# martenlienen/generative-turbulence

Measured on AMD Instinct MI355X. Metric: U-Net fwd+bwd voxels/sec (DDPM training step, 192x64x48x4), higher is better.
Workload: dtype bf16

## Files before the change

generative-turbulence_amd/csrc/tdx_resize.hip:

```cpp
#include "tdx_common.h"
#include <stdlib.h>

struct AxisMap {
    int in, out;
    float scale;
};
__host__ __device__ inline AxisMap make_axis(int in, int out) {
    AxisMap a;
    a.in = in; a.out = out;
    a.scale = out > 1 ? (float)(in - 1) / (float)(out - 1) : 0.0f;
    return a;
}
__host__ __device__ __forceinline__ void axis_taps(const AxisMap& a, int o, int& i0, int& i1, float& w1) {
    const float src = a.scale * (float)o;
    i0 = min((int)src, a.in - 1);
    w1 = fminf(fmaxf(src - (float)i0, 0.0f), 1.0f);
    i1 = i0 + ((i0 + 1 < a.in) ? 1 : 0);
}

struct TileGrid {
    int nx, ny, nz;
    int sy, sz;
    int tx, ty, tz;
};
// ... 184 lines not shown
__host__ __device__ __forceinline__ float axis_weight(const AxisMap& a, int o, int i) {
    int i0, i1;
    float w1;
    axis_taps(a, o, i0, i1, w1);
    float w = 0.f;
    if (i0 == i) w += 1.0f - w1;
    if (i1 == i) w += w1;
    return w;
}
__host__ __device__ __forceinline__ void axis_span(const AxisMap& a, int i, int& first, int& cnt) {
    int lo, hi;
    axis_range(a, i, lo, hi);
    first = hi + 1;
    int last = lo - 1;
    for (int o = lo; o <= hi; ++o)
        if (axis_weight(a, o, i) != 0.f) {
            first = min(first, o);
            last = o;
        }
    cnt = last - first + 1;
    if (cnt < 0) cnt = 0;
}

template <typename T, int K>
__global__ void __launch_bounds__(256)
resize_bwd_kernel(const T* __restrict__ dy, const T* __restrict__ add, T* __restrict__ dx, AxisMap ax, AxisMap ay, AxisMap az,
                  int C, TileGrid tg) {
    __shared__ int s_first[3][RS_MAXT], s_cnt[3][RS_MAXT];
    __shared__ float s_w[3][RS_MAXT][RS_KMAX];
    int b, ix0, iy0, iz0;
    tile_origin(tg, b, ix0, iy0, iz0);
    if (threadIdx.x < 3 * RS_MAXT) {
        const int a = threadIdx.x / RS_MAXT, k = threadIdx.x % RS_MAXT;
        const AxisMap& m = a == 0 ? ax : (a == 1 ? ay : az);
        const int i = min((a == 0 ? ix0 : (a == 1 ? iy0 : iz0)) + k, m.in - 1);
        int f, c;
        axis_span(m, i, f, c);
        s_first[a][k] = f; s_cnt[a][k] = c;
        for (int j = 0; j < RS_KMAX; ++j) s_w[a][k][j] = j < c ? axis_weight(m, f + j, i) : 0.f;
    }
    __syncthreads();
    const int L = C >> 3;
    const int per_pass = 256 / L;
    const int lc = (int)threadIdx.x % L;
    const int nvox = tg.tx * tg.ty * tg.tz;
    if ((int)threadIdx.x >= per_pass * L) return;
    for (int slot = (int)threadIdx.x / L; slot < nvox; slot += per_pass) {
        const int kz = slot & (tg.tz - 1), ky = (slot >> tg.sz) & (tg.ty - 1), kx = slot >> (tg.sz + tg.sy);
        const int ix = ix0 + kx, iy = iy0 + ky, iz = iz0 + kz;
        if (ix >= ax.in || iy >= ay.in || iz >= az.in) continue;
        const int fx = s_first[0][kx], cx = s_cnt[0][kx], fy = s_first[1][ky], cy = s_cnt[1][ky], fz = s_first[2][kz];
        float wz[K];
        int oz[K];
#pragma unroll
        for (int k = 0; k < K; ++k) {
            oz[k] = min(fz + k, az.out - 1);
            wz[k] = s_w[2][kz][k];
        }
        const T* gb = dy + ((int64_t)b * ax.out * ay.out * az.out) * C + lc * 8;
        float acc[8];
#pragma unroll
        for (int j = 0; j < 8; ++j) acc[j] = 0.f;
        for (int a = 0; a < cx; ++a) {
            const float wx = s_w[0][kx][a];
            for (int bb = 0; bb < cy; ++bb) {
                const float wxy = wx * s_w[1][ky][bb];
                const T* row = gb + (((int64_t)(fx + a) * ay.out + (fy + bb)) * az.out) * C;
                Raw8<T> t[K];
#pragma unroll
                for (int k = 0; k < K; ++k) t[k].load(row + (int64_t)oz[k] * C);
                __builtin_amdgcn_sched_barrier(0);
#pragma unroll
                for (int k = 0; k < K; ++k) {
                    const float w = wxy * wz[k];
                    const Vec8<T> v = t[k].get();
#pragma unroll
                    for (int j = 0; j < 8; ++j) acc[j] += w * v.v[j];
                }
            }
        }
        const int64_t di = ((((int64_t)b * ax.in + ix) * ay.in + iy) * az.in + iz) * C + lc * 8;
        if (add != nullptr) {
            Vec8<T> a;
            a.load(add + di);
#pragma unroll
            for (int j = 0; j < 8; ++j) acc[j] += a.v[j];
        }
        Vec8<T> o;
#pragma unroll
        for (int j = 0; j < 8; ++j) o.v[j] = acc[j];
        o.store(dx + di);
    }
}

template <typename T>
__global__ void __launch_bounds__(256)
resize_bwd_generic_kernel(const T* __restrict__ dy, const T* __restrict__ add, T* __restrict__ dx, AxisMap ax, AxisMap ay,
                          AxisMap az, int C, int64_t total) {
    const int L = C >> 3;
    int64_t i = (int64_t)blockIdx.x * blockDim.x + threadIdx.x;
    if (i >= total) return;
    const int lc = (int)(i % L);
    int64_t v = i / L;
    const int iz = (int)(v % az.in); v /= az.in;
    const int iy = (int)(v % ay.in); v /= ay.in;
// ... 65 lines not shown
    const AxisMap mx = make_axis(Xi, Xo), my = make_axis(Yi, Yo), mz = make_axis(Zi, Zo);
    if (C <= 64 && !((tg.tx | tg.ty | tg.tz) & 1) && Xo > Xi && Yo > Yi && Zo > Zi && pair_window_ok(mx) &&
        pair_window_ok(my) && pair_window_ok(mz)) {
        TDX_DISPATCH_DTYPE(dtype, hipLaunchKernelGGL((resize_up_pairs_kernel<T>), dim3((unsigned)blocks), dim3(256), 0,
                                                      as_stream(stream), (const T*)x, (T*)y, mx, my, mz, C, tg));
        return tdx_launch_status();
    }
    TDX_DISPATCH_DTYPE(dtype, hipLaunchKernelGGL((resize_fwd_kernel<T>), dim3((unsigned)blocks), dim3(256), 0,
                                                  as_stream(stream), (const T*)x, (T*)y, make_axis(Xi, Xo),
                                                  make_axis(Yi, Yo), make_axis(Zi, Zo), C, tg));
    return tdx_launch_status();
}

static int axis_max_span(const AxisMap& a) {
    int m = 0;
    for (int i = 0; i < a.in; ++i) {
        int f, c;
        axis_span(a, i, f, c);
        m = c > m ? c : m;
    }
    return m;
}

extern "C" int tdx_resize_bwd(const void* dy, const void* add, void* dx, int B, int Xi, int Yi, int Zi, int Xo, int Yo, int Zo, int C,
                              int dtype, void* stream) {
    TDX_CHECK_ARG(dy && dx && resize_args_ok(B, Xi, Yi, Zi, Xo, Yo, Zo, C));
    if (C % 8 || C / 8 > 256) return TDX_ESHAPE;
    const AxisMap ax = make_axis(Xi, Xo), ay = make_axis(Yi, Yo), az = make_axis(Zi, Zo);
    const int kx = axis_max_span(ax), ky = axis_max_span(ay), kz = axis_max_span(az);
    if (kx > RS_KMAX || ky > RS_KMAX || kz > RS_KMAX) {
        const int64_t total = (int64_t)B * Xi * Yi * Zi * (C / 8);
        TDX_DISPATCH_DTYPE(dtype, hipLaunchKernelGGL((resize_bwd_generic_kernel<T>), dim3(ceil_div(total, 256)), dim3(256), 0,
                                                      as_stream(stream), (const T*)dy, (const T*)add, (T*)dx, ax, ay, az, C, total));
        return tdx_launch_status();
    }
    const TileGrid tg = make_tiles(Xi, Yi, Zi, C, B);
    const dim3 grid((unsigned)((int64_t)B * tg.nx * tg.ny * tg.nz));
#define RS_BWD(KV)                                                                                                     \
    TDX_DISPATCH_DTYPE(dtype, hipLaunchKernelGGL((resize_bwd_kernel<T, KV>), grid, dim3(256), 0, as_stream(stream),     \
                                                  (const T*)dy, (const T*)add, (T*)dx, ax, ay, az, C, tg))
    if (kz <= 2) RS_BWD(2);
    else if (kz <= 4) RS_BWD(4);
    else if (kz <= 6) RS_BWD(6);
    else RS_BWD(RS_KMAX);
#undef RS_BWD
    return tdx_launch_status();
}
```

generative-turbulence_amd/turbdiff_amd/_lib.py:

```python

from __future__ import annotations

import ctypes as C
import os
import threading
from pathlib import Path

import torch

_HERE = Path(__file__).resolve().parent
LIB_PATH = Path(os.environ.get("TDX_LIB", _HERE / "libtdx_hip.so"))

F32, BF16 = 0, 1
F16 = 3
CONV_AUTO, CONV_DIRECT, CONV_MFMA, CONV_SPLIT = 0, 1, 2, 3
F32_SPLIT = 2
WS_CLEAN = 0x100

_vp, _i, _i64, _u64, _f, _sz = C.c_void_p, C.c_int, C.c_int64, C.c_uint64, C.c_float, C.c_size_t

SIGNATURES = {
    "tdx_version": (_i, []),
    "tdx_arch": (C.c_char_p, []),
    "tdx_set_scratch": (_i, [_vp, _sz]),
# ... 10 lines not shown
    "tdx_conv3_fwd_gn": (_i, [_vp, _i, _vp, _i, _vp, _vp, _vp, _vp, _i, _f, _vp, _i, _i, _i, _i, _i, _i, _i, _vp]),
    "tdx_conv3_fwd_partial": (_i, [_vp, _i, _i, _vp, _vp, _vp, _i, _vp, _vp, _i, _f, _vp, _i, _i, _i, _i, _i, _i, _i, _vp]),
    "tdx_conv3_bwd_data_workspace_bytes": (_sz, [_i, _i, _i, _i, _i, _i, _i]),
    "tdx_conv3_bwd_data": (_i, [_vp, _vp, _vp, _i, _vp, _i, _i, _i, _i, _i, _i, _i, _i, _i, _vp, _vp]),
    "tdx_conv3_bwd_data_add": (_i, [_vp, _vp, _vp, _i, _vp, _i, _vp, _vp, _i, _i, _i, _i, _i, _i, _i, _vp, _vp]),
    "tdx_conv3_bwd_weight_workspace_bytes": (_sz, [_i, _i, _i]),
    "tdx_conv3_bwd_weight": (_i, [_vp, _i, _vp, _i, _vp, _vp, _vp, _i, _i, _i, _i, _i, _i, _i, _vp, _vp]),
    "tdx_conv1_fwd": (_i, [_vp, _i, _vp, _i, _vp, _i, _vp, _vp, _vp, _i64, _i, _i, _vp]),
    "tdx_conv1_fwd_gn": (_i, [_vp, _i, _vp, _i, _vp, _i, _vp, _vp, _vp, _vp, _vp, _i, _vp, _i, _i64, _i, _i, _vp]),
    "tdx_conv1_bwd_weight": (_i, [_vp, _i, _vp, _i, _vp, _i, _vp, _i64, _i, _vp]),
    "tdx_conv1_bwd_weight_oc": (_i, [_vp, _i, _vp, _i, _vp, _i, _vp, _i, _i64, _i, _vp]),
    "tdx_encode_fwd": (_i, [_vp, _i, _vp, _vp, _vp, _i, _vp, _vp, _vp, _i, _i64, _i, _i, _vp]),
    "tdx_encode_bwd": (_i, [_vp, _vp, _i, _vp, _i, _vp, _vp, _vp, _vp, _vp, _vp, _i, _i64, _i, _i, _vp]),
    "tdx_decode_fwd": (_i, [_vp, _vp, _vp, _vp, _i, _i64, _i, _i, _i, _vp]),
    "tdx_decode_bwd": (_i, [_vp, _vp, _vp, _vp, _vp, _vp, _i, _i64, _i, _i, _i, _vp]),
    "tdx_gn_workspace_bytes": (_sz, [_i, _i]),
    "tdx_gn_stats": (_i, [_vp, _vp, _i, _i64, _i, _i, _f, _i, _vp, _vp]),
    "tdx_gn_apply": (_i, [_vp, _vp, _vp, _vp, _vp, _vp, _vp, _vp, _i, _i64, _i, _i, _i, _i, _vp]),
    "tdx_gn_apply_decode": (_i, [_vp, _vp, _vp, _vp, _vp, _vp, _vp, _vp, _i, _i64, _i, _i, _i, _i, _vp]),
    "tdx_gn_apply_encoded": (_i, [_vp, _vp, _vp, _vp, _vp, _i, _vp, _vp, _vp, _i, _vp, _vp, _vp, _i, _i64, _i, _i, _i, _vp]),
    "tdx_gn_bwd": (_i, [_vp] * 12 + [_i, _i64, _i, _i, _i, _i, _vp, _vp]),
    "tdx_resize_fwd": (_i, [_vp, _vp] + [_i] * 9 + [_vp]),
    "tdx_resize_bwd": (_i, [_vp, _vp, _vp] + [_i] * 9 + [_vp]),
    "tdx_attn_fwd": (_i, [_vp, _vp, _vp, _i, _i, _i, _i, _i, _vp]),
    "tdx_attn_bwd": (_i, [_vp, _vp, _vp, _vp, _vp, _i, _i, _i, _i, _i, _vp, _vp]),
    "tdx_attn_bwd_workspace_bytes": (_sz, [_i, _i, _i, _i]),
    "tdx_cell_mask": (_i, [_vp, _i64, _vp, _i64, _vp]),
    "tdx_q_sample": (_i, [_vp, _vp, _vp, _vp, _vp, _i, _vp, _i, _vp, _i, _i, _i64, _vp]),
    "tdx_p_sample_step": (_i, [_vp] * 7 + [_i, _vp, _i, _i, _vp, _i, _i, _i64, _vp]),
    "tdx_p_sample_step_rng": (_i, [_vp] * 5 + [_i, _vp, _i, _i, _vp, _i, _i, _i64, _u64, _vp, _vp, _vp]),
    "tdx_masked_loss": (_i, [_vp, _vp, _vp, _i64, _i, _vp, _vp, _i, _i, _i64, _vp, _vp]),
    "tdx_masked_loss_dyn": (_i, [_vp, _vp, _vp, _vp, _i, _vp, _vp, _i, _i, _i64, _vp, _vp]),
    "tdx_masked_loss_workspace_bytes": (_sz, []),
    "tdx_grid_embed": (_i, [_vp, _i, _vp, _i, _vp, _i, _vp, _i, _vp, _vp, _vp, _vp, _vp, _vp, _vp, _i, _i64, _i64, _vp]),
    "tdx_grid_select": (_i, [_vp, _vp, _vp, _vp, _vp, _i, _vp, _i, _vp, _i, _vp, _i, _i, _i64, _i64, _vp]),
    "tdx_cell_embed_fwd": (_i, [_vp, _vp, _vp, _i, _i, _i64, _vp]),
    "tdx_cell_embed_bwd_workspace_bytes": (_sz, [_i, _i]),
    "tdx_cell_embed_bwd": (_i, [_vp, _vp, _vp, _i, _i, _i, _i64, _vp, _vp]),
    "tdx_tke_energy": (_i, [_vp, _vp, _i, _i64, _vp]),
    "tdx_tke_sphere": (_i, [_vp, _vp, _vp, _vp, _vp, _i, _i, _i, _i, _i, _i, _vp]),
    "tdx_fd": (_i, [_vp, _vp, _i, _i, _i, _i, _f, _f, _f, _f, _i, _vp]),
    "tdx_ot_features": (_i, [_vp, _vp, _vp, _vp, _vp, _vp, _i, _i64, _i, _i, _i, _f, _f, _f, _vp]),
    "tdx_ot_workspace_bytes": (_sz, [_i, _i]),
    "tdx_ot_auction": (_i, [_vp, _vp, _i64, _vp, _vp, _i, _vp, _i, _i, _i, C.c_double, _i, _i64, _vp, _i, _i, _vp, _vp, _vp]),
    "tdx_randn": (_i, [_vp, _i64, _u64, _u64, _vp, _vp]),
    "tdx_randn_batched": (_i, [_vp, _i, _i64, _u64, _vp, _vp, _vp]),
# ... 275 lines not shown
```

generative-turbulence_amd/turbdiff_amd/models/ddpm.py:

```python

from __future__ import annotations

import math
import os
from dataclasses import dataclass
from functools import partial

import torch
import torch.nn.functional as F
from torch import nn

from .. import _lib, ops, schedules
from ..sequential import KwargsSequential
from .conditioning import global_conditioning, local_conditioning
from .utils import broadcast_right


@dataclass
class ModelPrediction:
    noise: torch.Tensor
    x_start: torch.Tensor
    mean: torch.Tensor
    log_var: torch.Tensor

# ... 55 lines not shown
        if self._fused_act:
            return ops.gn_film_silu(h, self.norm.weight, self.norm.bias, G, scale, shift, res=res, act=True,
                                    eps=self.norm.eps, stats=stats)
        h = ops.gn_film_silu(h, self.norm.weight, self.norm.bias, G, scale, shift, act=False, eps=self.norm.eps,
                             stats=stats)
        h = self.act(h)
        return h if res is None else h + res


class ResnetBlock(nn.Module):

    def __init__(self, dim_in, dim_out, *, c_dim: int, actfn, norm_klass):
        super().__init__()
        self.project_onto_scale_shift = nn.Linear(c_dim, dim_out * 2)
        self.block1 = Block(dim_in, dim_out, actfn=actfn, norm_klass=norm_klass)
        self.block2 = Block(dim_out, dim_out, actfn=actfn, norm_klass=norm_klass)
        self.conv = nn.Conv3d(dim_in, dim_out, 1) if dim_in != dim_out else nn.Identity()
        self.dim_out = dim_out

    def fused(self, x2=None):
        identity = isinstance(self.conv, nn.Identity)
        return self.block1._fused_act and self.block2._fused_act and not (identity and x2 is not None) and FUSE_BLOCKS

    def forward(self, x, c, x2=None, partial=None, conv1=None, films=None, skip_encoded=None, decode_wb=None):
        film = films.get(id(self)) if films is not None else None
        if film is None:
            film = ops.film_projections(c, [self.project_onto_scale_shift])[0]
        scale, shift = film[0], film[1]
        identity = isinstance(self.conv, nn.Identity)
        if self.fused(x2):
            b1, b2 = self.block1, self.block2
            if conv1 is not None:
                assert identity and x2 is None
                return ops.resnet_block(x, None, scale, shift, (conv1[1], conv1[2]), (b1.norm.weight, b1.norm.bias),
                                        (b2.conv.weight, b2.conv.bias), (b2.norm.weight, b2.norm.bias), None,
                                        _norm_groups(b1.norm), b1.norm.eps, conv1_input=conv1[0],
                                        conv1_real_channels=conv1[3] if len(conv1) > 3 else None, film=film,
                                        skip_encoded=skip_encoded)
            return ops.resnet_block(x, x2, scale, shift, (b1.conv.weight, b1.conv.bias), (b1.norm.weight, b1.norm.bias),
                                    (b2.conv.weight, b2.conv.bias), (b2.norm.weight, b2.norm.bias),
                                    None if identity else (self.conv.weight, self.conv.bias), _norm_groups(b1.norm),
                                    b1.norm.eps, partial=partial, film=film, decode_wb=decode_wb)
        assert partial is None and conv1 is None and skip_encoded is None and decode_wb is None
        h = self.block1(x, scale_shift=(scale, shift), x2=x2)
        if isinstance(self.conv, nn.Identity):
            skip = x if x2 is None else torch.cat((x, x2), dim=-1)
        else:
            skip = ops.conv1(x, self.conv.weight, self.conv.bias, x2=x2)
        return self.block2(h, res=skip)


class Attention(nn.Module):
# ... 44 lines not shown
        super().__init__()
        assert len(downsampling_blocks) == len(upsampling_blocks)
        self.downsampling_blocks = nn.ModuleList(downsampling_blocks)
        self.upsampling_blocks = nn.ModuleList(upsampling_blocks)
        self.center_block = center_block
        self.downsampling_factor = downsampling_factor
        self.scale_factor = 1 / downsampling_factor

    def forward(self, x, c, first_partial=None, first_conv=None, films=None, first_skip=None):
        skips = []
        assert first_skip is None or first_conv is not None
        for i, blk in enumerate(self.downsampling_blocks):
            if i == 0 and first_conv is not None:
                x = blk(x, c, conv1=first_conv, films=films, skip_encoded=first_skip)
            elif i == 0 and first_partial is not None:
                x = blk(x, c, partial=first_partial, films=films)
            else:
                x = blk(x, c, films=films)
            skip, x = ops.skip_and_resize(x, [max(int(s * self.scale_factor), 3) for s in x.shape[1:4]])
            skips.append(skip)
        x = self.center_block(x, c=c, films=films)
        for blk in self.upsampling_blocks:
            skip = skips.pop()
            x = blk(ops.resize(x, skip.shape[1:4]), c, x2=skip, films=films)
        return x


class GeometryEmbedding(nn.Module):

    def __init__(self, in_features, out_features, actfn):
        super().__init__()
        self.in_features, self.out_features, self.actfn = in_features, out_features, actfn
        self.extract_features = nn.Sequential(
            nn.Conv3d(in_features, out_features, kernel_size=5, stride=5),
            actfn(),
            nn.Conv3d(out_features, out_features, kernel_size=5, stride=1),
            actfn(),
            nn.Conv3d(out_features, out_features, kernel_size=5, stride=5),
        )

    def forward(self, c_local):
        front = torch.narrow(c_local, dim=-3, start=0, length=50)
        return self.extract_features(front).mean(dim=(-3, -2, -1))




# ... 542 lines not shown
```

generative-turbulence_amd/turbdiff_amd/ops.py:

```python

from __future__ import annotations

import weakref

import os

import torch
from torch.autograd.function import once_differentiable

from . import _lib as L


def _ws(nbytes: int, device) -> torch.Tensor:
    return torch.empty(max(int(nbytes), 16), dtype=torch.uint8, device=device)


_CLEAN = {}
WS_CLEAN = 0 if os.environ.get("TDX_WS_CLEAN", "1") == "0" else L.WS_CLEAN


def _clean_ws(nbytes: int, device, tag=None) -> torch.Tensor:
    if not WS_CLEAN:
        return _ws(nbytes, device)
    key = (device, L.stream(device.index), int(nbytes), tag)
# ... 97 lines not shown

def _gn_bwd(x, gy, stats, gamma, beta, scale, shift, dscale, dshift, B, V, Cc, groups, act, code, st, ws=None):
    gx, dgamma, dbeta = torch.empty_like(x), stats.new_empty(Cc), stats.new_empty(Cc)
    if ws is None:
        ws = _gn_ws(B, Cc, x.device)
    L.call("tdx_gn_bwd", L.ptr(x), L.ptr(gy), L.ptr(stats), L.ptr(gamma), L.ptr(beta), L.ptr(scale), L.ptr(shift), L.ptr(gx),
           L.ptr(dgamma), L.ptr(dbeta), L.ptr(dscale), L.ptr(dshift), B, V, Cc, groups, act, code, L.ptr(ws), st)
    return gx, dgamma, dbeta


def _resize_fwd(x, size):
    B, Xi, Yi, Zi, Cc = _grid(x)
    Xo, Yo, Zo = (int(s) for s in size)
    y = torch.empty((B, Xo, Yo, Zo, Cc), dtype=x.dtype, device=x.device)
    L.call("tdx_resize_fwd", L.ptr(x), L.ptr(y), B, Xi, Yi, Zi, Xo, Yo, Zo, Cc, L.dtype_code(x.dtype), L.stream())
    return y, (B, Xi, Yi, Zi, Xo, Yo, Zo, Cc)


def _resize_bwd(gy, add, geom):
    B, Xi, Yi, Zi, Xo, Yo, Zo, Cc = geom
    gx = torch.empty((B, Xi, Yi, Zi, Cc), dtype=gy.dtype, device=gy.device)
    L.call("tdx_resize_bwd", L.ptr(gy), L.ptr(add), L.ptr(gx), B, Xi, Yi, Zi, Xo, Yo, Zo, Cc, L.dtype_code(gy.dtype), L.stream())
    return gx




class _ToNVC(torch.autograd.Function):

    @staticmethod
    def forward(ctx, x, dtype):
        ctx.in_dtype = x.dtype
        return _to_nvc(x.contiguous(), dtype)

    @staticmethod
    @once_differentiable
    def backward(ctx, gy):
        return _to_ncv(gy.contiguous(), ctx.in_dtype), None


class _ToNCV(torch.autograd.Function):

    @staticmethod
    def forward(ctx, x, dtype):
        ctx.in_dtype = x.dtype
        return _to_ncv(x.contiguous(), dtype)
# ... 268 lines not shown
        return gx1, gx2, gw, gb, None, None


def conv3(x1, weight, bias=None, x2=None):
    return _Conv3.apply(x1, x2, weight, bias)


def conv3_gn_stats(x1, weight, bias, groups, eps=1e-5, x2=None):
    return _Conv3.apply(x1, x2, weight, bias, groups, eps)




def _conv1_wt(weight: torch.Tensor) -> torch.Tensor:
    key = (id(weight), "wt")
    hit = _cached(key, weight)
    if hit is not None:
        return hit[0]
    wt = weight.detach().reshape(weight.shape[0], -1).t().contiguous()
    _cache_store(key, weight, wt)
    return wt


def _conv1_weight_grad(x1, C1, x2, C2, gy, Cout, has_bias, rows, code, st):
    Cin = C1 + C2
    off = (Cout * Cin + 63) // 64 * 64
    buf = torch.zeros(off + (Cout if has_bias else 0), dtype=torch.float32, device=gy.device)
    gw = buf[: Cout * Cin].view(Cout, Cin)
    gb = buf[off:] if has_bias else None
    L.call("tdx_conv1_bwd_weight_oc", L.ptr(x1), C1, L.ptr(gy), Cout, gw.data_ptr(), Cin, L.ptr(gb), 1, rows, code, st)
    if x2 is not None:
        L.call("tdx_conv1_bwd_weight_oc", L.ptr(x2), C2, L.ptr(gy), Cout, gw.data_ptr() + 4 * C1, Cin, None, 1, rows, code, st)
    return gw, gb


class _Conv1(torch.autograd.Function):
    @staticmethod
    def forward(ctx, x1, x2, weight, bias, add):
        C1 = x1.shape[-1]
        C2 = 0 if x2 is None else x2.shape[-1]
        Cout = weight.shape[0]
        w2 = weight.detach().reshape(Cout, -1)
        assert w2.shape[1] == C1 + C2
        x1 = x1.contiguous()
        x2 = None if x2 is None else x2.contiguous()
        add = None if add is None else add.contiguous()
        lead = tuple(x1.shape[:-1])
        y = _conv1_fwd(x1, C1, x2, C2, _conv1_wt(weight), Cout, 0, bias, add, lead, x1.numel() // C1, Cout,
                       L.dtype_code(x1.dtype), L.stream())
        ctx.save_for_backward(x1, x2, w2.contiguous())
        ctx.has_bias = bias is not None
        ctx.has_add = add is not None
        ctx.wshape = tuple(weight.shape)
        return y

# ... 288 lines not shown


def film_projections(c: torch.Tensor, linears) -> list:
    B, T = c.shape
    if not L.query("tdx_film_supported", B, T):
        out = []
        for lin in linears:
            f = torch.nn.functional.linear(c.float(), lin.weight.float(), lin.bias.float())
            out.append(torch.stack(f.chunk(2, dim=1)))
        return out
    args = []
    for lin in linears:
        args += [lin.weight, lin.bias]
    return list(_FilmProjections.apply(c, *args))




_SIDE = {}


FUSE_SKIP_TAIL = True
WGRAD_STREAM = os.environ.get("TDX_WGRAD_STREAM", "1") != "0"


class _WgradSide:

    def __init__(self, device):
        self.on = WGRAD_STREAM
        self.pending = False
        if self.on:
            idx = device.index
            if idx not in _SIDE:
                _SIDE[idx] = torch.cuda.Stream(device=device, priority=int(os.environ.get("TDX_WGRAD_STREAM_PRIORITY", "0")))
                L.declare_zero_block_only(_SIDE[idx])
            self.side, self.main = _SIDE[idx], torch.cuda.current_stream(device)

    def run(self, fn, *tensors):
        if not self.on:
            return fn()
        for t in tensors:
            if t is not None:
                t.record_stream(self.side)
        self.side.wait_stream(self.main)
        self.pending = True
        with torch.cuda.stream(self.side):
            fn()

    def join(self):
        if self.on and self.pending:
            self.main.wait_stream(self.side)
            self.pending = False


class _ResnetBlock(torch.autograd.Function):

    @staticmethod
    def forward(ctx, x1, x2, film, w1, b1, g1, be1, w2, b2, g2, be2, wr, br, groups, eps, partial=None, xc=None,
                xc_real=None, enc=None, dec=None):
        B, X, Y, Z, C1 = x1.shape if enc is not None else _grid(x1)
        C2 = 0 if x2 is None else x2.shape[-1]
        Cin, Cout = C1 + C2, w1.shape[0]
        if xc is not None:
            assert x2 is None and wr is None and partial is None and xc.shape[:4] == x1.shape[:4] and xc.dtype == x1.dtype
            xc = xc.contiguous()
        if enc is not None:
            assert xc is not None and wr is None and C1 == Cout
        Cc = xc.shape[-1] if xc is not None else Cin
        assert w1.shape[1] == Cc
        V = X * Y * Z
        dev, dt = x1.device, x1.dtype
        code, impl, st = L.dtype_code(dt), L.conv_impl(), L.stream()
        x1 = x1.contiguous() if enc is None else None
        x2 = None if x2 is None else x2.contiguous()
        wf1, wb1 = _packed_conv3(w1, dt)
        wf2, wb2 = _packed_conv3(w2, dt)
        f32c = lambda t: t.detach().float().contiguous()
        g1, be1, g2, be2 = f32c(g1), f32c(be1), f32c(g2), f32c(be2)
        film = f32c(film.reshape(2, B, Cout))
        scale, shift = film[0], film[1]
        grid, gn, gws = (B, X, Y, Z), (groups, eps), _gn_ws(B, Cout, dev, clean=True)

# ... 19 lines not shown
            F = wd.shape[0]
            out = torch.empty((B, F, X, Y, Z), dtype=torch.float32, device=dev)
            L.call("tdx_gn_apply_decode", L.ptr(h2), L.ptr(st2), L.ptr(g2), L.ptr(be2), L.ptr(x1),
                   L.ptr(wd.detach().reshape(F, Cout).float().contiguous()), L.ptr(bd.detach().float().contiguous()), L.ptr(out),
                   B, V, Cout, groups, F, code, st)
            return out
        if enc is not None:
            xr, Fx, wx2, bx2, cr, Fc, wc2, bc2, D = enc
            y = torch.empty_like(h1)
            L.call("tdx_gn_apply_encoded", L.ptr(h2), L.ptr(st2), L.ptr(g2), L.ptr(be2), L.ptr(xr), Fx, L.ptr(wx2), L.ptr(bx2),
                   L.ptr(cr), Fc, L.ptr(wc2), L.ptr(bc2), L.ptr(y), B, V, D, groups, code, st)
        elif wr is None:
            assert x2 is None and Cin == Cout
            y = _gn_apply(h2, st2, g2, be2, None, None, x1, B, V, Cout, groups, 1, code, st)
        else:
            wr2 = wr.detach().reshape(Cout, Cin).contiguous()
            if FUSE_SKIP_TAIL and dt in L.H16_DTYPES and C1 % 32 == 0 and C2 % 32 == 0 and Cout % 32 == 0:
                y = torch.empty_like(h1)
                L.call("tdx_conv1_fwd_gn", L.ptr(x1), C1, L.ptr(x2), C2, L.ptr(_conv1_wt(wr)), Cout, L.ptr(br), L.ptr(h2),
                       L.ptr(st2), L.ptr(g2), L.ptr(be2), groups, L.ptr(y), B, V, Cout, code, st)
            else:
                res = _conv1_fwd(x1, C1, x2, C2, _conv1_wt(wr), Cout, 0, br, None, grid, B * V, Cout, code, st)
                y = _gn_apply(h2, st2, g2, be2, None, None, res, B, V, Cout, groups, 1, code, st)
        ctx.save_for_backward(x1, x2, h1, st1, a1, h2, st2, film, g1, be1, g2, be2, wb1, wb2, wr2, xc)
        ctx.cfg = (groups, tuple(w1.shape), tuple(w2.shape), None if wr is None else tuple(wr.shape),
                   b1 is not None, b2 is not None, br is not None)
        ctx.xc_real, ctx.impl, ctx.c1 = xc_real, impl, C1
        return y

    @staticmethod
    @once_differentiable
    def backward(ctx, gy):
        side = _WgradSide(gy.device)
        try:
            return _ResnetBlock._backward(ctx, gy, side)
        finally:
            side.join()

    @staticmethod
    def _backward(ctx, gy, side):
        x1, x2, h1, st1, a1, h2, st2, film, g1, be1, g2, be2, wb1, wb2, wr2, xc = ctx.saved_tensors
        scale, shift = film[0], film[1]
        groups, w1s, w2s, wrs, hb1, hb2, hbr = ctx.cfg
        B, X, Y, Z, _ = _grid(h1)
        C1 = ctx.c1
        C2 = 0 if x2 is None else x2.shape[-1]
        Cin, Cout = C1 + C2, w1s[0]
        Cc = w1s[1]
        grid, V = (B, X, Y, Z), X * Y * Z
        gy = gy.contiguous()
        dev, code, impl, st = gy.device, L.dtype_code(gy.dtype), ctx.impl, L.stream()
        gws = _gn_ws(B, Cout, dev)

        dh2, dg2, dbe2 = _gn_bwd(h2, gy, st2, g2, be2, None, None, None, None, B, V, Cout, groups, 1, code, st, gws)
        dw2, db2 = _conv3_wgrad_out(w2s, hb2, dev)
        wws2, wws1 = _conv3_wgrad_ws(Cout, Cout, impl, dev), _conv3_wgrad_ws(Cc, Cout, impl, dev)
        side.run(lambda: _conv3_wgrad(a1, Cout, None, 0, dh2, dw2, db2, grid, Cout, code, impl, wws2, L.stream()), a1, dh2, dw2, db2)
        dws = _conv3_bwd_data_ws(grid, max(Cin, Cout, Cc), code, impl, dev)
        da1, _ = _conv3_bwd_data(dh2, wb2, a1, Cout, None, 0, grid, Cout, code, impl, st, dws)
        del dh2
        dfilm = torch.empty((2, B, Cout), dtype=torch.float32, device=dev)
        dh1, dg1, dbe1 = _gn_bwd(h1, da1, st1, g1, be1, scale, shift, dfilm[0], dfilm[1], B, V, Cout, groups, 1, code, st, gws)
        del da1
        dw1, db1 = _conv3_wgrad_out(w1s, hb1, dev)
        if xc is not None:
            real = ctx.xc_real
            side.run(lambda: _conv3_wgrad(xc, Cc, None, 0, dh1, dw1, db1, grid, Cout, code, impl, wws1, L.stream(), real),
                     xc, dh1, dw1, db1)
            dxc = None
            if ctx.needs_input_grad[16]:
                dxc, _ = _conv3_bwd_data(dh1, wb1, xc, Cc, None, 0, grid, Cout, code, impl, st, dws, real=real)
            side.join()
            return (gy, None, dfilm, dw1, db1, dg1, dbe1, dw2, db2, dg2, dbe2, None, None, None, None, None, dxc, None, None,
                    None)
        side.run(lambda: _conv3_wgrad(x1, C1, x2, C2, dh1, dw1, db1, grid, Cout, code, impl, wws1, L.stream()),
                 x1, x2, dh1, dw1, db1)
        dwr = dbr = None
        if wr2 is None:
            gx1, gx2 = _conv3_bwd_data(dh1, wb1, x1, C1, None, 0, grid, Cout, code, impl, st, dws, add=gy)
        else:
            t1, t2 = _conv3_bwd_data(dh1, wb1, x1, C1, x2, C2, grid, Cout, code, impl, st, dws)
            gx1 = _conv1_fwd(gy, Cout, None, 0, wr2, Cin, 0, None, t1, grid, B * V, C1, code, st)
            gx2 = None if x2 is None else _conv1_fwd(gy, Cout, None, 0, wr2, Cin, C1, None, t2, grid, B * V, C2, code, st)
            dwr, dbr = _conv1_weight_grad(x1, C1, x2, C2, gy, Cout, hbr, B * V, code, st)
            dwr = dwr.view(wrs)
        side.join()
        return (gx1, gx2, dfilm, dw1, db1, dg1, dbe1, dw2, db2, dg2, dbe2, dwr, dbr, None, None, None, None, None, None, None)


def resnet_block(x1, x2, scale, shift, conv1_wb, norm1_wb, conv2_wb, norm2_wb, skip_wb, groups, eps=1e-5, partial=None,
                 conv1_input=None, conv1_real_channels=None, film=None, skip_encoded=None, decode_wb=None):
    wr, br = skip_wb if skip_wb is not None else (None, None)
    assert decode_wb is None or not torch.is_grad_enabled(), "decode_wb: inference only (the block output is not kept)"
    assert partial is None or not torch.is_grad_enabled(), "partial: inference only (the backward needs the full conv)"
    enc = None
    if skip_encoded is not None:
        assert x1 is skip_encoded.standin and conv1_input is not None and skip_wb is None and x2 is None
        enc = skip_encoded.operands
    if film is None:
        B, Cout = x1.shape[0], conv1_wb[0].shape[0]
        film = torch.stack((scale.reshape(B, Cout).float(), shift.reshape(B, Cout).float()))
    return _ResnetBlock.apply(x1, x2, film, conv1_wb[0], conv1_wb[1], norm1_wb[0], norm1_wb[1], conv2_wb[0],
                              conv2_wb[1], norm2_wb[0], norm2_wb[1], wr, br, groups, eps, partial, conv1_input,
                              conv1_real_channels, enc, decode_wb)




def _taps_first(w5: torch.Tensor, in_axis: int, out_axis: int) -> torch.Tensor:
    k = w5.shape[-1]
# ... 101 lines not shown
```

include/tdx.h:

```cpp
#ifndef TDX_H
#define TDX_H

#include <stddef.h>
#include <stdint.h>

#ifdef __cplusplus
extern "C" {
#endif

#define TDX_F32 0
#define TDX_BF16 1

#define TDX_OK 0
#define TDX_EINVAL (-1)
#define TDX_ESHAPE (-2)
#define TDX_EDTYPE (-3)

#define TDX_CONV_AUTO 0
#define TDX_CONV_DIRECT 1
#define TDX_CONV_MFMA 2
#define TDX_CONV_SPLIT 3
#define TDX_F32_SPLIT 2
#define TDX_F16 3
#define TDX_WS_CLEAN 0x100
// ... 71 lines not shown
int tdx_decode_bwd(const float* dy, const void* h, const float* w, void* dh, float* dw, float* db, int B, int64_t V, int D,
                   int F, int dtype, void* stream);

size_t tdx_gn_workspace_bytes(int B, int C);
int tdx_gn_stats(const void* x, float* stats, int B, int64_t V, int C, int G, float eps, int dtype, void* workspace,
                 void* stream);
int tdx_gn_apply(const void* x, const float* stats, const float* gamma, const float* beta, const float* scale,
                 const float* shift, const void* res, void* y, int B, int64_t V, int C, int G, int act, int dtype,
                 void* stream);
int tdx_gn_apply_encoded(const void* x, const float* stats, const float* gamma, const float* beta, const float* x_raw, int Fx,
                         const float* wx, const float* bx, const float* c_raw, int Fc, const float* wc, const float* bc,
                         void* y, int B, int64_t V, int D, int G, int dtype, void* stream);
int tdx_gn_apply_decode(const void* x, const float* stats, const float* gamma, const float* beta, const void* res,
                        const float* w, const float* bias, float* out, int B, int64_t V, int C, int G, int F, int dtype,
                        void* stream);
int tdx_gn_bwd(const void* x, const void* dy, const float* stats, const float* gamma, const float* beta,
               const float* scale, const float* shift, void* dx, float* dgamma, float* dbeta, float* dscale,
               float* dshift, int B, int64_t V, int C, int G, int act, int dtype, void* workspace, void* stream);

int tdx_resize_fwd(const void* x, void* y, int B, int Xi, int Yi, int Zi, int Xo, int Yo, int Zo, int C, int dtype,
                   void* stream);
int tdx_resize_bwd(const void* dy, const void* add, void* dx, int B, int Xi, int Yi, int Zi, int Xo, int Yo, int Zo, int C,
                   int dtype, void* stream);

int tdx_attn_fwd(const void* qkv, void* out, float* lse, int B, int N, int H, int D, int dtype, void* stream);
int tdx_attn_bwd(const void* qkv, const void* out, const float* lse, const void* dout, void* dqkv, int B, int N, int H,
                 int D, int dtype, void* workspace, void* stream);
size_t tdx_attn_bwd_workspace_bytes(int B, int N, int H, int D);


int tdx_cell_mask(const int64_t* cell_idx, int64_t n_cells, uint8_t* mask, int64_t V, void* stream);

int tdx_q_sample(const float* x0, const float* noise, const float* sqrt_ac, const float* sqrt_1mac, const int64_t* t,
                 int t_stride, const uint8_t* mask, int keep_bcs, float* out, int B, int F, int64_t V, void* stream);

int tdx_p_sample_step(const float* x_t, const float* eps, const float* z, const float* z2, const float* x_bcs,
                      const uint8_t* mask, const float* sched, int T, const int64_t* t, int noise_bcs, int clip,
                      float* out, int B, int F, int64_t V, void* stream);

int tdx_p_sample_step_rng(const float* x_t, const float* eps, const float* x_bcs, const uint8_t* mask, const float* sched,
                          int T, int64_t* t, int noise_bcs, int clip, float* out, int B, int F, int64_t V, uint64_t seed,
                          const uint64_t* stream_ids, uint64_t* offset_dev, void* stream);

int tdx_masked_loss(const float* eps_hat, const float* noise, const uint8_t* mask, int64_t n_cells, int l1,
                    float* loss, float* grad, int B, int F, int64_t V, void* workspace, void* stream);
int tdx_masked_loss_dyn(const float* eps_hat, const float* noise, const unsigned char* mask, const int64_t* n_cells_dev,
// ... 123 lines not shown
```

Before: 169.6 million.

## Fuse upsample into up-block backward and run skip 1x1 conv at coarse resolution

Adds an _UpBlock autograd function that resizes the coarse input inside the resnet block and saves the coarse tensor. In backward it resizes both the conv3 data gradient and the output gradient down to coarse resolution in one paired kernel (tdx_resize_bwd2). The skip 1x1 conv data and weight gradients for the upsampled branch then run on coarse voxels, relying on linearity of interpolation to commute with the 1x1 conv. This removes a separate resize backward pass and shrinks the 1x1 work, at the cost of an extra resize of gy and more complex bookkeeping, and results may differ numerically from the original order.

```diff
diff --git a/generative-turbulence_amd/csrc/tdx_resize.hip b/generative-turbulence_amd/csrc/tdx_resize.hip
--- a/generative-turbulence_amd/csrc/tdx_resize.hip
+++ b/generative-turbulence_amd/csrc/tdx_resize.hip
@@ -230,10 +230,10 @@
     if (cnt < 0) cnt = 0;
 }
 
-template <typename T, int K>
+template <typename T, int K, bool PAIR>
 __global__ void __launch_bounds__(256)
-resize_bwd_kernel(const T* __restrict__ dy, const T* __restrict__ add, T* __restrict__ dx, AxisMap ax, AxisMap ay, AxisMap az,
-                  int C, TileGrid tg) {
+resize_bwd_kernel(const T* __restrict__ dy, const T* __restrict__ add, T* __restrict__ dx, const T* __restrict__ dy_b,
+                  T* __restrict__ dx_b, AxisMap ax, AxisMap ay, AxisMap az, int C, int Cb, TileGrid tg) {
     __shared__ int s_first[3][RS_MAXT], s_cnt[3][RS_MAXT];
     __shared__ float s_w[3][RS_MAXT][RS_KMAX];
     int b, ix0, iy0, iz0;
@@ -248,11 +248,15 @@
         for (int j = 0; j < RS_KMAX; ++j) s_w[a][k][j] = j < c ? axis_weight(m, f + j, i) : 0.f;
     }
     __syncthreads();
-    const int L = C >> 3;
+    const int L = (C + (PAIR ? Cb : 0)) >> 3;
     const int per_pass = 256 / L;
-    const int lc = (int)threadIdx.x % L;
+    int lc = (int)threadIdx.x % L;
     const int nvox = tg.tx * tg.ty * tg.tz;
     if ((int)threadIdx.x >= per_pass * L) return;
+    if (PAIR && lc >= (C >> 3)) {
+        lc -= C >> 3;
+        dy = dy_b; dx = dx_b; C = Cb;
+    }
     for (int slot = (int)threadIdx.x / L; slot < nvox; slot += per_pass) {
         const int kz = slot & (tg.tz - 1), ky = (slot >> tg.sz) & (tg.ty - 1), kx = slot >> (tg.sz + tg.sy);
         const int ix = ix0 + kx, iy = iy0 + ky, iz = iz0 + kz;
@@ -288,7 +292,7 @@
             }
         }
         const int64_t di = ((((int64_t)b * ax.in + ix) * ay.in + iy) * az.in + iz) * C + lc * 8;
-        if (add != nullptr) {
+        if (!PAIR && add != nullptr) {
             Vec8<T> a;
             a.load(add + di);
 #pragma unroll
@@ -400,27 +404,52 @@
     return m;
 }
 
-extern "C" int tdx_resize_bwd(const void* dy, const void* add, void* dx, int B, int Xi, int Yi, int Zi, int Xo, int Yo, int Zo, int C,
-                              int dtype, void* stream) {
-    TDX_CHECK_ARG(dy && dx && resize_args_ok(B, Xi, Yi, Zi, Xo, Yo, Zo, C));
-    if (C % 8 || C / 8 > 256) return TDX_ESHAPE;
+static int resize_bwd_launch(const void* dy, const void* add, void* dx, int C, const void* dy_b, void* dx_b, int Cb, int B, int Xi,
+                             int Yi, int Zi, int Xo, int Yo, int Zo, int dtype, void* stream) {
     const AxisMap ax = make_axis(Xi, Xo), ay = make_axis(Yi, Yo), az = make_axis(Zi, Zo);
     const int kx = axis_max_span(ax), ky = axis_max_span(ay), kz = axis_max_span(az);
     if (kx > RS_KMAX || ky > RS_KMAX || kz > RS_KMAX) {
-        const int64_t total = (int64_t)B * Xi * Yi * Zi * (C / 8);
-        TDX_DISPATCH_DTYPE(dtype, hipLaunchKernelGGL((resize_bwd_generic_kernel<T>), dim3(ceil_div(total, 256)), dim3(256), 0,
-                                                      as_stream(stream), (const T*)dy, (const T*)add, (T*)dx, ax, ay, az, C, total));
+        const void* dys[2] = {dy, dy_b};
+        void* dxs[2] = {dx, dx_b};
+        const int Cs[2] = {C, Cb};
+        for (int i = 0; i < (dy_b ? 2 : 1); ++i) {
+            const int64_t total = (int64_t)B * Xi * Yi * Zi * (Cs[i] / 8);
+            TDX_DISPATCH_DTYPE(dtype, hipLaunchKernelGGL((resize_bwd_generic_kernel<T>), dim3(ceil_div(total, 256)), dim3(256), 0,
+                                                          as_stream(stream), (const T*)dys[i], (const T*)(i ? nullptr : add),
+                                                          (T*)dxs[i], ax, ay, az, Cs[i], total));
+        }
         return tdx_launch_status();
     }
-    const TileGrid tg = make_tiles(Xi, Yi, Zi, C, B);
+    const TileGrid tg = make_tiles(Xi, Yi, Zi, C + Cb, B);
     const dim3 grid((unsigned)((int64_t)B * tg.nx * tg.ny * tg.nz));
+#define RS_BWD2(KV, PV)                                                                                                     \
+    TDX_DISPATCH_DTYPE(dtype, hipLaunchKernelGGL((resize_bwd_kernel<T, KV, PV>), grid, dim3(256), 0, as_stream(stream),      \
+                                                  (const T*)dy, (const T*)add, (T*)dx, (const T*)dy_b, (T*)dx_b, ax, ay, az, C, \
+                                                  Cb, tg))
 #define RS_BWD(KV)                                                                                                     \
-    TDX_DISPATCH_DTYPE(dtype, hipLaunchKernelGGL((resize_bwd_kernel<T, KV>), grid, dim3(256), 0, as_stream(stream),     \
-                                                  (const T*)dy, (const T*)add, (T*)dx, ax, ay, az, C, tg))
+    do {                                                                                                               \
+        if (dy_b) RS_BWD2(KV, true);                                                                                   \
+        else RS_BWD2(KV, false);                                                                                       \
+    } while (0)
     if (kz <= 2) RS_BWD(2);
     else if (kz <= 4) RS_BWD(4);
     else if (kz <= 6) RS_BWD(6);
     else RS_BWD(RS_KMAX);
 #undef RS_BWD
+#undef RS_BWD2
     return tdx_launch_status();
 }
+
+extern "C" int tdx_resize_bwd(const void* dy, const void* add, void* dx, int B, int Xi, int Yi, int Zi, int Xo, int Yo, int Zo, int C,
+                              int dtype, void* stream) {
+    TDX_CHECK_ARG(dy && dx && resize_args_ok(B, Xi, Yi, Zi, Xo, Yo, Zo, C));
+    if (C % 8 || C / 8 > 256) return TDX_ESHAPE;
+    return resize_bwd_launch(dy, add, dx, C, nullptr, nullptr, 0, B, Xi, Yi, Zi, Xo, Yo, Zo, dtype, stream);
+}
+
+extern "C" int tdx_resize_bwd2(const void* dy_a, int Ca, const void* dy_b, int Cb, void* dx_a, void* dx_b, int B, int Xi, int Yi,
+                               int Zi, int Xo, int Yo, int Zo, int dtype, void* stream) {
+    TDX_CHECK_ARG(dy_a && dy_b && dx_a && dx_b && Cb > 0 && resize_args_ok(B, Xi, Yi, Zi, Xo, Yo, Zo, Ca));
+    if (Ca % 8 || Cb % 8 || (Ca + Cb) / 8 > 256) return TDX_ESHAPE;
+    return resize_bwd_launch(dy_a, nullptr, dx_a, Ca, dy_b, dx_b, Cb, B, Xi, Yi, Zi, Xo, Yo, Zo, dtype, stream);
+}
diff --git a/generative-turbulence_amd/turbdiff_amd/_lib.py b/generative-turbulence_amd/turbdiff_amd/_lib.py
--- a/generative-turbulence_amd/turbdiff_amd/_lib.py
+++ b/generative-turbulence_amd/turbdiff_amd/_lib.py
@@ -56,6 +56,7 @@
     "tdx_gn_bwd": (_i, [_vp] * 12 + [_i, _i64, _i, _i, _i, _i, _vp, _vp]),
     "tdx_resize_fwd": (_i, [_vp, _vp] + [_i] * 9 + [_vp]),
     "tdx_resize_bwd": (_i, [_vp, _vp, _vp] + [_i] * 9 + [_vp]),
+    "tdx_resize_bwd2": (_i, [_vp, _i, _vp, _i, _vp, _vp] + [_i] * 8 + [_vp]),
     "tdx_attn_fwd": (_i, [_vp, _vp, _vp, _i, _i, _i, _i, _i, _vp]),
     "tdx_attn_bwd": (_i, [_vp, _vp, _vp, _vp, _vp, _i, _i, _i, _i, _i, _vp, _vp]),
     "tdx_attn_bwd_workspace_bytes": (_sz, [_i, _i, _i, _i]),
diff --git a/generative-turbulence_amd/turbdiff_amd/models/ddpm.py b/generative-turbulence_amd/turbdiff_amd/models/ddpm.py
--- a/generative-turbulence_amd/turbdiff_amd/models/ddpm.py
+++ b/generative-turbulence_amd/turbdiff_amd/models/ddpm.py
@@ -101,12 +101,19 @@
         identity = isinstance(self.conv, nn.Identity)
         return self.block1._fused_act and self.block2._fused_act and not (identity and x2 is not None) and FUSE_BLOCKS
 
-    def forward(self, x, c, x2=None, partial=None, conv1=None, films=None, skip_encoded=None, decode_wb=None):
+    def forward(self, x, c, x2=None, partial=None, conv1=None, films=None, skip_encoded=None, decode_wb=None, upsample=False):
         film = films.get(id(self)) if films is not None else None
         if film is None:
             film = ops.film_projections(c, [self.project_onto_scale_shift])[0]
         scale, shift = film[0], film[1]
         identity = isinstance(self.conv, nn.Identity)
+        if upsample:
+            if self.fused(x2) and not identity:
+                b1, b2 = self.block1, self.block2
+                return ops.up_block(x, x2, scale, shift, (b1.conv.weight, b1.conv.bias), (b1.norm.weight, b1.norm.bias),
+                                    (b2.conv.weight, b2.conv.bias), (b2.norm.weight, b2.norm.bias),
+                                    (self.conv.weight, self.conv.bias), _norm_groups(b1.norm), b1.norm.eps, film=film)
+            x = ops.resize(x, x2.shape[1:4])
         if self.fused(x2):
             b1, b2 = self.block1, self.block2
             if conv1 is not None:
@@ -197,7 +204,7 @@
         x = self.center_block(x, c=c, films=films)
         for blk in self.upsampling_blocks:
             skip = skips.pop()
-            x = blk(ops.resize(x, skip.shape[1:4]), c, x2=skip, films=films)
+            x = blk(x, c, x2=skip, films=films, upsample=True)
         return x
 
 
diff --git a/generative-turbulence_amd/turbdiff_amd/ops.py b/generative-turbulence_amd/turbdiff_amd/ops.py
--- a/generative-turbulence_amd/turbdiff_amd/ops.py
+++ b/generative-turbulence_amd/turbdiff_amd/ops.py
@@ -143,6 +143,16 @@
     gx = torch.empty((B, Xi, Yi, Zi, Cc), dtype=gy.dtype, device=gy.device)
     L.call("tdx_resize_bwd", L.ptr(gy), L.ptr(add), L.ptr(gx), B, Xi, Yi, Zi, Xo, Yo, Zo, Cc, L.dtype_code(gy.dtype), L.stream())
     return gx
+
+
+def _resize_bwd2(gy_a, gy_b, geom):
+    B, Xi, Yi, Zi, Xo, Yo, Zo, _ = geom
+    Ca, Cb = gy_a.shape[-1], gy_b.shape[-1]
+    gx_a = torch.empty((B, Xi, Yi, Zi, Ca), dtype=gy_a.dtype, device=gy_a.device)
+    gx_b = torch.empty((B, Xi, Yi, Zi, Cb), dtype=gy_a.dtype, device=gy_a.device)
+    L.call("tdx_resize_bwd2", L.ptr(gy_a), Ca, L.ptr(gy_b), Cb, L.ptr(gx_a), L.ptr(gx_b), B, Xi, Yi, Zi, Xo, Yo, Zo,
+           L.dtype_code(gy_a.dtype), L.stream())
+    return gx_a, gx_b
 
 
 
@@ -457,15 +467,20 @@
     return wt
 
 
-def _conv1_weight_grad(x1, C1, x2, C2, gy, Cout, has_bias, rows, code, st):
+def _conv1_weight_grad(x1, C1, x2, C2, gy, Cout, has_bias, rows, code, st, x2_gy=None, x2_rows=None):
     Cin = C1 + C2
     off = (Cout * Cin + 63) // 64 * 64
     buf = torch.zeros(off + (Cout if has_bias else 0), dtype=torch.float32, device=gy.device)
     gw = buf[: Cout * Cin].view(Cout, Cin)
     gb = buf[off:] if has_bias else None
-    L.call("tdx_conv1_bwd_weight_oc", L.ptr(x1), C1, L.ptr(gy), Cout, gw.data_ptr(), Cin, L.ptr(gb), 1, rows, code, st)
+    if x2_gy is None or x2 is None:
+        x2_gy, x2_rows, gb1, gb2 = gy, rows, gb, None
+    else:
+        gb1, gb2 = None, gb
+    L.call("tdx_conv1_bwd_weight_oc", L.ptr(x1), C1, L.ptr(gy), Cout, gw.data_ptr(), Cin, L.ptr(gb1), 1, rows, code, st)
     if x2 is not None:
-        L.call("tdx_conv1_bwd_weight_oc", L.ptr(x2), C2, L.ptr(gy), Cout, gw.data_ptr() + 4 * C1, Cin, None, 1, rows, code, st)
+        L.call("tdx_conv1_bwd_weight_oc", L.ptr(x2), C2, L.ptr(x2_gy), Cout, gw.data_ptr() + 4 * C1, Cin, L.ptr(gb2), 1, x2_rows,
+               code, st)
     return gw, gb
 
 
@@ -800,6 +815,7 @@
 
 FUSE_SKIP_TAIL = True
 WGRAD_STREAM = os.environ.get("TDX_WGRAD_STREAM", "1") != "0"
+UP_BLOCK = os.environ.get("TDX_UP_BLOCK", "1") != "0"
 
 
 class _WgradSide:
@@ -835,7 +851,8 @@
 
     @staticmethod
     def forward(ctx, x1, x2, film, w1, b1, g1, be1, w2, b2, g2, be2, wr, br, groups, eps, partial=None, xc=None,
-                xc_real=None, enc=None, dec=None):
+                xc_real=None, enc=None, dec=None, up=None):
+        assert up is None or (wr is not None and xc is None and partial is None and dec is None)
         B, X, Y, Z, C1 = x1.shape if enc is not None else _grid(x1)
         C2 = 0 if x2 is None else x2.shape[-1]
         Cin, Cout = C1 + C2, w1.shape[0]
@@ -901,7 +918,8 @@
             else:
                 res = _conv1_fwd(x1, C1, x2, C2, _conv1_wt(wr), Cout, 0, br, None, grid, B * V, Cout, code, st)
                 y = _gn_apply(h2, st2, g2, be2, None, None, res, B, V, Cout, groups, 1, code, st)
-        ctx.save_for_backward(x1, x2, h1, st1, a1, h2, st2, film, g1, be1, g2, be2, wb1, wb2, wr2, xc)
+        ctx.save_for_backward(x1, x2, h1, st1, a1, h2, st2, film, g1, be1, g2, be2, wb1, wb2, wr2, xc, None if up is None else up[0])
+        ctx.up_geom = None if up is None else up[1]
         ctx.cfg = (groups, tuple(w1.shape), tuple(w2.shape), None if wr is None else tuple(wr.shape),
                    b1 is not None, b2 is not None, br is not None)
         ctx.xc_real, ctx.impl, ctx.c1 = xc_real, impl, C1
@@ -910,6 +928,10 @@
     @staticmethod
     @once_differentiable
     def backward(ctx, gy):
+        return _ResnetBlock._joined_backward(ctx, gy)
+
+    @staticmethod
+    def _joined_backward(ctx, gy):
         side = _WgradSide(gy.device)
         try:
             return _ResnetBlock._backward(ctx, gy, side)
@@ -918,7 +940,7 @@
 
     @staticmethod
     def _backward(ctx, gy, side):
-        x1, x2, h1, st1, a1, h2, st2, film, g1, be1, g2, be2, wb1, wb2, wr2, xc = ctx.saved_tensors
+        x1, x2, h1, st1, a1, h2, st2, film, g1, be1, g2, be2, wb1, wb2, wr2, xc, x_c = ctx.saved_tensors
         scale, shift = film[0], film[1]
         groups, w1s, w2s, wrs, hb1, hb2, hbr = ctx.cfg
         B, X, Y, Z, _ = _grid(h1)
@@ -959,12 +981,47 @@
             gx1, gx2 = _conv3_bwd_data(dh1, wb1, x1, C1, None, 0, grid, Cout, code, impl, st, dws, add=gy)
         else:
             t1, t2 = _conv3_bwd_data(dh1, wb1, x1, C1, x2, C2, grid, Cout, code, impl, st, dws)
-            gx1 = _conv1_fwd(gy, Cout, None, 0, wr2, Cin, 0, None, t1, grid, B * V, C1, code, st)
-            gx2 = None if x2 is None else _conv1_fwd(gy, Cout, None, 0, wr2, Cin, C1, None, t2, grid, B * V, C2, code, st)
-            dwr, dbr = _conv1_weight_grad(x1, C1, x2, C2, gy, Cout, hbr, B * V, code, st)
+            if x_c is None:
+                gx1 = _conv1_fwd(gy, Cout, None, 0, wr2, Cin, 0, None, t1, grid, B * V, C1, code, st)
+                gx2 = None if x2 is None else _conv1_fwd(gy, Cout, None, 0, wr2, Cin, C1, None, t2, grid, B * V, C2, code, st)
+                dwr, dbr = _conv1_weight_grad(x1, C1, x2, C2, gy, Cout, hbr, B * V, code, st)
+            else:
+                gx2 = None if x2 is None else _conv1_fwd(gy, Cout, None, 0, wr2, Cin, C1, None, t2, grid, B * V, C2, code, st)
+                r_c, g_c = _resize_bwd2(t1, gy, ctx.up_geom)
+                cgrid = tuple(x_c.shape[:4])
+                rows_c = x_c.numel() // C1
+                gx1 = _conv1_fwd(g_c, Cout, None, 0, wr2, Cin, 0, None, r_c, cgrid, rows_c, C1, code, st)
+                dwr, dbr = _conv1_weight_grad(x_c, C1, x2, C2, g_c, Cout, hbr, rows_c, code, st, x2_gy=gy, x2_rows=B * V)
             dwr = dwr.view(wrs)
         side.join()
         return (gx1, gx2, dfilm, dw1, db1, dg1, dbe1, dw2, db2, dg2, dbe2, dwr, dbr, None, None, None, None, None, None, None)
+
+
+class _UpBlock(torch.autograd.Function):
+
+    @staticmethod
+    def forward(ctx, x_c, x2, film, w1, b1, g1, be1, w2, b2, g2, be2, wr, br, groups, eps, size):
+        x_c = x_c.contiguous()
+        x1, geom = _resize_fwd(x_c, size)
+        return _ResnetBlock.forward(ctx, x1, x2, film, w1, b1, g1, be1, w2, b2, g2, be2, wr, br, groups, eps, up=(x_c, geom))
+
+    @staticmethod
+    @once_differentiable
+    def backward(ctx, gy):
+        return _ResnetBlock._joined_backward(ctx, gy)[:15] + (None,)
+
+
+def up_block(x_coarse, skip, scale, shift, conv1_wb, norm1_wb, conv2_wb, norm2_wb, skip_wb, groups, eps=1e-5, film=None):
+    size = tuple(skip.shape[1:4])
+    C1, Cout = x_coarse.shape[-1], conv1_wb[0].shape[0]
+    if not UP_BLOCK or skip_wb is None or C1 % 8 or Cout % 8 or (C1 + Cout) // 8 > 256:
+        return resnet_block(resize(x_coarse, size), skip, scale, shift, conv1_wb, norm1_wb, conv2_wb, norm2_wb, skip_wb, groups,
+                            eps, film=film)
+    if film is None:
+        B = x_coarse.shape[0]
+        film = torch.stack((scale.reshape(B, Cout).float(), shift.reshape(B, Cout).float()))
+    return _UpBlock.apply(x_coarse, skip, film, conv1_wb[0], conv1_wb[1], norm1_wb[0], norm1_wb[1], conv2_wb[0], conv2_wb[1],
+                          norm2_wb[0], norm2_wb[1], skip_wb[0], skip_wb[1], groups, eps, size)
 
 
 def resnet_block(x1, x2, scale, shift, conv1_wb, norm1_wb, conv2_wb, norm2_wb, skip_wb, groups, eps=1e-5, partial=None,
diff --git a/include/tdx.h b/include/tdx.h
--- a/include/tdx.h
+++ b/include/tdx.h
@@ -117,6 +117,8 @@
                    void* stream);
 int tdx_resize_bwd(const void* dy, const void* add, void* dx, int B, int Xi, int Yi, int Zi, int Xo, int Yo, int Zo, int C,
                    int dtype, void* stream);
+int tdx_resize_bwd2(const void* dy_a, int Ca, const void* dy_b, int Cb, void* dx_a, void* dx_b, int B, int Xi, int Yi, int Zi,
+                    int Xo, int Yo, int Zo, int dtype, void* stream);
 
 int tdx_attn_fwd(const void* qkv, void* out, float* lse, int B, int N, int H, int D, int dtype, void* stream);
 int tdx_attn_bwd(const void* qkv, const void* out, const float* lse, const void* dout, void* dqkv, int B, int N, int H,
```

Result: no change. 169.3 million (median of 2 runs) (-0.2%).
